# alevar/tiebrush

Measured on AMD Instinct MI355X. Metric: input alignment records/sec collapsed (tiebrush) + bases/sec covered (tiecov), higher is better.
Workload: dtype int64; 1 GPU; c3: 64 synthetic sorted BAMs x 5000000 100bp reads per GPU, --clip collapse + tiecov -c -j of the result; records_per_gpu=320000000, groups_out=25086541, parallelism=files-per-rank x1, ranks_seen=1, resident=SoA in HBM before the timed region, contexts=3

## Files before the change

### tiebrush_amd/csrc/collapse.hip

```cpp
#include <stdlib.h>

#include <chrono>

#include "cb_tiles.hpp"
#include "dev_common.hpp"
#include "rx_w64.hpp"
#include "scan_op.hpp"
#include "strategy.hpp"
#include "tbk_internal.h"
#include "wgroup.h"

namespace {

struct EffKey {
  uint32_t khi_h, khi_l;
  int32_t kend;
  uint32_t flag_cnt;
};
struct EffOp {
  __device__ __forceinline__ EffKey operator()(const EffKey& a, const EffKey& b) const {
    uint64_t ak = ((uint64_t)a.khi_h << 32) | a.khi_l, bk = ((uint64_t)b.khi_h << 32) | b.khi_l;
    bool take_b = (b.flag_cnt >> 31) || bk > ak || (bk == ak && b.kend > a.kend);
    EffKey r;
    r.khi_h = take_b ? b.khi_h : a.khi_h;
// ... 1915 lines not shown
      if (n_long && !literal) {
        hipStream_t keep = ctx->stream;
        if (aux) ctx->stream = aux;
        TBK_LAUNCH(ctx, "yd_wave", yd_wave_k, n_long, 64, 0, ids_long, n_wave, nchains, nit, chain_first, Y, YdWords{iv, io}, noff, ex_s, ex_e, J.g_yd,
                   yd_d, ids_over, n_over);
        ctx->stream = keep;
        if (aux) TBK_HIP(hipEventRecord(ctx->aux_done, aux));
      }
      if (n_lane && !literal)
        TBK_LAUNCH(ctx, "yd_lane", yd_lane_k<8>, cdiv(n_lane, 64), 64, 0, ids_lane, n_lane, nchains, nit, chain_first, Y, YdWords{iv, io}, ex_s, ex_e, J.g_yd,
                   yd_d, ids_over, n_over);
      if (n_long && aux) TBK_HIP(hipStreamWaitEvent(ctx->stream, ctx->aux_done, 0));
      TBK_LAUNCH(ctx, "yd_run_overflow", yd_run_k, cdiv(nchains, 64), 64, 0, ids_over, n_over, nchains, nit, chain_first, Y, YdWords{iv, io}, noff, ex_s, ex_e,
                 N, J.g_yd, yd_d);
    }
    if (by_list) {
      TBK_LAUNCH(ctx, "yd_gather", yd_lgather_k, ys_tiles, 512, 0, ng, ys_tiles, ys_table, ys_totals, yd_d, ys_item, J.gperm, J.G, J.cap, J.out_yd);
      TBK_HIP(hipStreamSynchronize(ctx->stream));
      if (ph)
        fprintf(stderr, "YD stage ms: counts %.1f | placement + numbering %.1f | buckets %.1f | list machines + gather %.1f (arena %.2f of %.2f GB, %zu overflow chunks)\n",
                std::chrono::duration<double, std::milli>(p1 - p0).count(), std::chrono::duration<double, std::milli>(p2 - p1).count(),
                std::chrono::duration<double, std::milli>(p3 - p2).count(), since(p3), ctx->ws_off / 1e9, ctx->ws_cap / 1e9, ctx->ws_overflow.size());
      return tbk_check_launch(ctx, "collapse_yd");
    }
  }
  TBK_LAUNCH(ctx, "col_write_yd", col_write_yd_k, cdiv(ng, B), B, 0, ng, J.gperm, J.G, J.g_yd, J.cap, J.out_yd);
  TBK_HIP(hipStreamSynchronize(ctx->stream));
  return tbk_check_launch(ctx, "collapse_yd");
}

int tbk_collapse_warm(tbk_ctx* ctx) {
  TBK_HIP(hipSetDevice(ctx->device));
  uint64_t* sc = ctx->d_scalars;
  TBK_HIP(hipMemsetAsync(sc, 0, 32 * sizeof(uint64_t), ctx->stream));
  TBK_HIP(hipStreamSynchronize(ctx->stream));
  uint32_t* z = (uint32_t*)sc;
  YdItems Y{};
  Y.pk = (uint4*)sc, Y.nex = z;
  const YdWords W{nullptr, z};
  const SegNodes N{z, z, (int32_t*)z};
  hipStream_t aux = tbk_aux_stream(ctx);
  if (aux) {
    hipStream_t keep = ctx->stream;
    ctx->stream = aux;
    TBK_LAUNCH(ctx, "yd_wave", yd_wave_k, 1, 64, 0, z, z, 0u, 0u, z, Y, W, z, z, z, (int32_t*)nullptr, z + 8, z + 16, z + 1);
    ctx->stream = keep;
    TBK_HIP(hipEventRecord(ctx->aux_done, aux));
    TBK_HIP(hipStreamWaitEvent(ctx->stream, ctx->aux_done, 0));
  } else {
    TBK_LAUNCH(ctx, "yd_wave", yd_wave_k, 1, 64, 0, z, z, 0u, 0u, z, Y, W, z, z, z, (int32_t*)nullptr, z + 8, z + 16, z + 1);
  }
  TBK_LAUNCH(ctx, "yd_lane", yd_lane_k<8>, 1, 64, 0, z, 0u, 0u, 0u, z, Y, W, z, z, (int32_t*)nullptr, z + 8, z + 16, z + 1);
  TBK_LAUNCH(ctx, "yd_run_overflow", yd_run_k, 1, 64, 0, z, z, 0u, 0u, z, Y, W, z, z, z, N, (int32_t*)nullptr, z + 8);
  TBK_HIP(hipStreamSynchronize(ctx->stream));
  return tbk_check_launch(ctx, "warmup");
}

int tbk_collapse_device(tbk_ctx* ctx, const tbk_collapse_opts* o, const tbk_soa_in* in, tbk_groups_out* out) {
  const uint32_t n = in->n_records;
  const uint32_t B = 256;
  out->n_groups = 0;
  out->n_passed = 0;
  ctx->route = tbk_collapse_route{};
  if (out->rec_group) TBK_HIP(hipMemsetAsync(out->rec_group, 0xFF, (size_t)n * 4, ctx->stream));
  if (n == 0) return 0;
  uint64_t* sc = ctx->d_scalars;
  ColIn I;
  I.n = n;
  I.k = in->n_files;
  {
    uint32_t* d_fo = ws_alloc<uint32_t>(ctx, in->n_files + 1);
    uint8_t* d_tb = ws_alloc<uint8_t>(ctx, in->n_files);
    if (!d_fo || !d_tb) return TBK_ENOMEM;
    const size_t fo_bytes = (size_t)(in->n_files + 1) * 4, tb_bytes = in->n_files;
    if (fo_bytes + tb_bytes <= 4096 * sizeof(uint64_t)) {
      char* stage = (char*)tbk_stage_acquire(ctx);
      memcpy(stage, in->file_off, fo_bytes);
      TBK_HIP(hipMemcpyAsync(d_fo, stage, fo_bytes, hipMemcpyHostToDevice, ctx->stream));
      if (in->tbmerged) {
        memcpy(stage + fo_bytes, in->tbmerged, tb_bytes);
        TBK_HIP(hipMemcpyAsync(d_tb, stage + fo_bytes, tb_bytes, hipMemcpyHostToDevice, ctx->stream));
      } else {
        TBK_HIP(hipMemsetAsync(d_tb, 0, tb_bytes, ctx->stream));
      }
      tbk_stage_release(ctx);
    } else {
      TBK_HIP(hipMemcpyAsync(d_fo, in->file_off, fo_bytes, hipMemcpyHostToDevice, ctx->stream));
      if (in->tbmerged) {
        TBK_HIP(hipMemcpyAsync(d_tb, in->tbmerged, tb_bytes, hipMemcpyHostToDevice, ctx->stream));
      } else {
        TBK_HIP(hipMemsetAsync(d_tb, 0, tb_bytes, ctx->stream));
      }
      TBK_HIP(hipStreamSynchronize(ctx->stream));
    }
    I.file_off = d_fo;
    I.tbm = d_tb;
  }
  I.tid = in->tid;
  I.pos = in->pos;
  I.flag = in->flag;
  I.mapq = in->mapq;
  I.strand = in->strand;
  I.nh = in->nh;
  I.cig_off = in->cig_off;
  I.cig = in->cig;
  I.yc_in = in->yc_in;
// ... 771 lines not shown
```

### tiebrush_amd/csrc/tbk_api.hip

```cpp
#include <sys/mman.h>

#include <algorithm>
#include <chrono>
#include <mutex>
#include <vector>
#include <new>

#include "tbk_internal.h"

namespace {
std::mutex g_reg_m;
struct RegEntry {
  void* p;
  int users;
};
std::vector<RegEntry> g_reg;
}

static void release_registered(tbk_ctx* ctx) {
  if (ctx->registered.empty()) return;
  (void)hipStreamSynchronize(ctx->stream);
  const auto r0 = std::chrono::steady_clock::now();
  struct RP {
    tbk_ctx* c;
// ... 401 lines not shown
}

static int yd_stage_on(tbk_ctx* run_on, void* job, size_t hint) {
  if (hipSetDevice(run_on->device) != hipSuccess) return TBK_EHIP;
  tbk_prof_begin_call(run_on);
  int rc = ws_begin_call(run_on, hint);
  if (rc == 0) rc = tbk_collapse_yd_run(run_on, job);
  tbk_prof_end_call(run_on);
  return rc;
}

static int finish_yd(tbk_ctx* ctx) {
  if (!ctx->yd_pending) return 0;
  ctx->yd_worker->wait();
  ctx->yd_pending = false;
  ctx->ws_base_off = 0;
  if (ctx->yd_ctx) {
    ctx->last_times = ctx->yd_ctx->last_times;
    if (ctx->yd_rc != 0) ctx->last_error = ctx->yd_ctx->last_error;
  }
  return ctx->yd_rc;
}

void tbk_debug_parse(const char* spec, TbkDebug* out) {
  *out = TbkDebug();
  if (!spec) return;
  std::string s(spec);
  size_t at = 0;
  while (at < s.size()) {
    size_t end = s.find(',', at);
    if (end == std::string::npos) end = s.size();
    const std::string kv = s.substr(at, end - at);
    at = end + 1;
    const size_t eq = kv.find('=');
    const std::string k = kv.substr(0, eq), v = eq == std::string::npos ? std::string("1") : kv.substr(eq + 1);
    const unsigned long long u = strtoull(v.c_str(), nullptr, 0);
    const bool on = v != "0";
    if (k == "path") out->path = v == "sort" ? 1 : (v == "window" ? 2 : 0);
    else if (k == "raw") out->raw = on ? 1 : 0;
    else if (k == "sort") out->sort = v == "radix" ? 1 : (v == "runs" ? 2 : 0);
    else if (k == "scan") out->scan = v == "lookback" ? 1 : (v == "3pass" ? 2 : 0);
    else if (k == "hash_mask") out->hash_mask = (uint32_t)u;
    else if (k == "qhash_mask") out->qhash_mask = u;
    else if (k == "yd_wave_min") out->yd_wave_min = (uint32_t)u;
    else if (k == "yd_bgrid") out->yd_bgrid = (uint32_t)u;
    else if (k == "yd_radix") out->yd_radix = on;
    else if (k == "yd_literal") out->yd_literal = on;
    else if (k == "yd_front") out->yd_front_split = v == "split";
    else if (k == "yd_own_arena") out->yd_own_arena = on;
    else if (k == "wg_stats") out->wg_stats = on;
    else if (k == "wg_og") out->wg_og = (uint32_t)u;
    else if (k == "wg_dense_verify") out->wg_dense_verify = on;
    else if (k == "wg_rank_merge") out->wg_rank_merge = on;
    else if (k == "cov_legacy") out->cov_legacy = on;
    else if (k == "cov_bundle_scan") out->cov_bundle_scan = on;
    else if (k == "cov_prep") out->cov_prep = on;
    else if (k == "cov_tile_cap") out->cov_tile_cap = u;
    else if (k == "junc_radix") out->junc_radix = on;
    else if (k == "no_junc_agg") out->no_junc_agg = on;
    else if (k == "jh_cap") out->jh_cap = (uint32_t)u;
    else if (k == "index_chain") out->index_chain = on;
    else if (k == "no_register") out->no_register = on;
    else if (k == "phases") out->phases = on;
    else if (k == "no_bounce") out->no_bounce = on;
    else if (k == "fmt_slice") out->fmt_slice = u;
  }
}

extern "C" {

int tbk_abi_version(void) { return TBK_ABI_VERSION; }

int tbk_set_debug(tbk_ctx* ctx, const char* spec) {
  if (!ctx) return TBK_EINVAL;
  tbk_debug_parse(spec, &ctx->dbg);
  if (ctx->yd_ctx) ctx->yd_ctx->dbg = ctx->dbg;
  if (ctx->side_ctx) ctx->side_ctx->dbg = ctx->dbg;
  return 0;
}

const char* tbk_strerror(int s) {
  switch (s) {
    case TBK_OK: return "ok";
    case TBK_EINVAL: return "invalid argument";
    case TBK_ENOMEM: return "out of memory";
    case TBK_EHIP: return "HIP runtime error";
    case TBK_E2BIG: return "output capacity too small";
    case TBK_EUNSUPPORTED: return "option or input outside the supported/pinned semantics";
    case TBK_EUNSORTED: return "input not coordinate-sorted";
    case TBK_EFATALOP: return "unknown opcode (tiecov accepts only M/I/D/N/S)";
    case TBK_ECOLLISION: return "key hash collision survived all reseeds";
    case TBK_ENODEVICE: return "no usable gfx950 device";
  }
  return "unknown status";
}

int tbk_create(int device_ordinal, tbk_ctx** out) {
  if (!out) return TBK_EINVAL;
  *out = nullptr;
  int ndev = 0;
  if (hipGetDeviceCount(&ndev) != hipSuccess || ndev <= 0 || device_ordinal < 0 || device_ordinal >= ndev) return TBK_ENODEVICE;
  tbk_ctx* ctx = new (std::nothrow) tbk_ctx();
  if (!ctx) return TBK_ENOMEM;
  ctx->device = device_ordinal;
  tbk_debug_parse(getenv("TBK_DEBUG"), &ctx->dbg);
  bool ok = hipSetDevice(device_ordinal) == hipSuccess;
// ... 476 lines not shown
```

### tiebrush_amd/csrc/tbk_internal.h

```cpp
#pragma once
#include <hip/hip_runtime.h>
#include <stdint.h>
#include <stdio.h>
#include <string.h>

#include <string>
#include <condition_variable>
#include <functional>
#include <mutex>
#include <thread>
#include <utility>
#include <vector>

#include "../../include/tbk.h"

enum : uint32_t {
  TBK_DERR_UNSORTED = 1u << 0,
  TBK_DERR_COLLISION = 1u << 1,
  TBK_DERR_FATALOP = 1u << 2,
  TBK_DERR_SPAN = 1u << 3,
  TBK_DERR_NCIGAR = 1u << 4,
  TBK_DERR_FRACTIONAL = 1u << 5,
  TBK_DERR_OVERFLOW = 1u << 6,
  TBK_DERR_INTERNAL = 1u << 7,
// ... 17 lines not shown
      std::lock_guard<std::mutex> lk(m);
      if (!started) {
        started = true;
        th = std::thread([this]() {
          std::unique_lock<std::mutex> lk2(m);
          for (;;) {
            cv.wait(lk2, [&] { return quit || (bool)job; });
            if (quit) return;
            std::function<void()> run = std::move(job);
            job = nullptr;
            lk2.unlock();
            run();
            lk2.lock();
            busy = false;
            cv.notify_all();
          }
        });
      }
      job = std::move(j);
      busy = true;
    }
    cv.notify_all();
  }
  void wait() {
    std::unique_lock<std::mutex> lk(m);
    cv.wait(lk, [&] { return !busy; });
  }
  ~TbkWorker() {
    {
      std::lock_guard<std::mutex> lk(m);
      quit = true;
    }
    cv.notify_all();
    if (th.joinable()) th.join();
  }
};

struct TbkDebug {
  int path = 0;
  int raw = -1;
  int sort = 0;
  int scan = 0;
  uint32_t hash_mask = 0xFFFFFFFFu;
  uint64_t qhash_mask = ~0ull;
  uint32_t yd_wave_min = 0;
  uint32_t yd_bgrid = 0;
  bool yd_radix = false;
  bool yd_literal = false;
  bool yd_front_split = false;
  bool yd_own_arena = false;
  uint32_t wg_og = 0;
  bool wg_stats = false;
  bool wg_dense_verify = false, wg_rank_merge = false;
  bool cov_legacy = false, cov_bundle_scan = false, cov_prep = false, junc_radix = false, no_junc_agg = false;
  uint64_t cov_tile_cap = 0;
  uint32_t jh_cap = 0;
  bool index_chain = false;
  bool no_register = false;
  bool no_bounce = false;
  bool phases = false;
  uint64_t fmt_slice = 0;
};
void tbk_debug_parse(const char* spec, TbkDebug* out);

struct tbk_ctx {
  int device = 0;
  TbkDebug dbg;
  hipStream_t own_stream = nullptr;
  hipStream_t stream = nullptr;
  hipStream_t aux = nullptr;
  hipEvent_t aux_done = nullptr;
  char* ws = nullptr;
  size_t ws_cap = 0, ws_off = 0;
  size_t ws_top = 0;
  bool ws_top_mode = false;
  bool ws_borrowed = false;
  std::vector<std::pair<char*, size_t>> ws_overflow;
  size_t ws_over_used = 0;
  uint32_t* d_err = nullptr;
  uint64_t* d_scalars = nullptr;
  uint64_t* h_scalars = nullptr;
  hipEvent_t stage_ev = nullptr;
  char* d_view = nullptr;
  size_t d_view_cap = 0;
  struct ViewPrep {
    bool valid = false;
    const void* cig = nullptr;
    uint32_t n = 0;
    int32_t *start = nullptr, *end = nullptr, *yi = nullptr;
    uint32_t *jcnt = nullptr, *ridx = nullptr;
    const void* agg = nullptr;
    uint32_t agg_tiles = 0;
    uint64_t n_bases = 0, sum_abs = 0, n_junc = 0;
    uint32_t err = 0;
  } view_prep;
  bool profiling = false;
  std::vector<KTime> ktimes;
  std::vector<hipEvent_t> ev_pool;
  size_t ev_used = 0;
  std::vector<tbk_kernel_time> last_times;
  std::string last_error;
  tbk_collapse_route route{};
  int num_cu = 256;
  void* yd_job = nullptr;
  tbk_ctx* yd_ctx = nullptr;
  TbkWorker* yd_worker = nullptr;
// ... 72 lines not shown
template <class T>
static inline T* ws_alloc(tbk_ctx* ctx, size_t n) {
  return (T*)tbk_ws_alloc_raw(ctx, n * sizeof(T));
}

hipEvent_t tbk_event(tbk_ctx* ctx);
static inline void tbk_prof_begin(tbk_ctx* ctx, const char* name) {
  if (!ctx->profiling) return;
  KTime k{name, tbk_event(ctx), tbk_event(ctx)};
  (void)hipEventRecord(k.a, ctx->stream);
  ctx->ktimes.push_back(k);
}
static inline void tbk_prof_end(tbk_ctx* ctx) {
  if (!ctx->profiling) return;
  (void)hipEventRecord(ctx->ktimes.back().b, ctx->stream);
}

#define TBK_LAUNCH(ctx, name, kern, grid, block, shmem, ...)                          \
  do {                                                                                \
    tbk_prof_begin(ctx, name);                                                        \
    hipLaunchKernelGGL(kern, dim3(grid), dim3(block), shmem, (ctx)->stream, __VA_ARGS__); \
    tbk_prof_end(ctx);                                                                \
  } while (0)

void tbk_prof_begin_call(tbk_ctx* ctx);
void tbk_prof_end_call(tbk_ctx* ctx);
int tbk_check_launch(tbk_ctx* ctx, const char* what);
extern "C" void tbk_bam_release(tbk_ctx* ctx);
void* tbk_stage_acquire(tbk_ctx* ctx);
void tbk_stage_release(tbk_ctx* ctx);
int tbk_sync_err(tbk_ctx* ctx, uint32_t* err_bits);
int tbk_derr_to_status(tbk_ctx* ctx, uint32_t bits);

static inline uint32_t cdiv(uint64_t a, uint64_t b) { return (uint32_t)((a + b - 1) / b); }

int tbk_exscan_u32(tbk_ctx* ctx, const uint32_t* in, uint32_t* out, uint32_t n, uint64_t* d_total);
int tbk_exscan_u32_u64(tbk_ctx* ctx, const uint32_t* in, uint64_t* out, uint32_t n, uint64_t* d_total);

struct SortBufs {
  uint64_t *hi, *lo;
  uint32_t* val;
  uint64_t *hi2, *lo2;
  uint32_t* val2;
};
int tbk_radix_sort128(tbk_ctx* ctx, SortBufs* b, uint32_t n, uint64_t only_hi = ~0ull, uint64_t only_lo = ~0ull,
                      bool masks_are_exact = false);
size_t tbk_radix_ws_bytes(uint32_t n);
int tbk_radix_sort_w64(tbk_ctx* ctx, uint64_t** w, uint64_t** w2, uint32_t n, uint64_t mask, bool mask_is_exact);
int tbk_sort_runs(tbk_ctx* ctx, SortBufs* b, uint32_t n_hi, const uint32_t* d_run_off, uint32_t nruns, uint32_t* err,
                  uint32_t* nbig_zeroed);

int tbk_collapse_device(tbk_ctx* ctx, const tbk_collapse_opts* o, const tbk_soa_in* in, tbk_groups_out* out);
int tbk_collapse_warm(tbk_ctx* ctx);
int tbk_collapse_yd_run(tbk_ctx* run_on, void* job);
int tbk_coverage_device(tbk_ctx* ctx, const tbk_cov_in* in, tbk_cov_out* out);
int tbk_cov_view_build(tbk_ctx* ctx, const int32_t* r_tid, const int32_t* r_pos, const uint8_t* r_strand, const uint32_t* r_cig_off,
                       const uint32_t* r_cig, const uint32_t* g_rep, const double* g_yc, const int64_t* g_yx, uint32_t ng, tbk_cov_in* view,
                       const uint64_t* g_key = nullptr);
int tbk_sample_device(tbk_ctx* ctx, const tbk_cov_in* in, int32_t num_samples, tbk_sample_out* out);
int tbk_format_device(tbk_ctx* ctx, const tbk_track_rows* rows, tbk_track_sink sink, void* user, uint64_t* out_bytes);
int tbk_names_upload(tbk_ctx* ctx, uint32_t n_names, const uint64_t* off, const char* bytes);
```

### tiebrush_amd/csrc/wgroup.hip

```cpp
#include <stdlib.h>

#include <algorithm>

#include "dev_common.hpp"
#include "strategy.hpp"
#include "tbk_internal.h"
#include "wgroup.h"

namespace {

constexpr int WG_NT = 512;
constexpr int WG_E = 8;
constexpr int WG_CAP = WG_NT * WG_E;
constexpr uint32_t WG_T = 1024;
constexpr uint32_t WG_KS = 2048;
constexpr int WG_NW = WG_NT / 64;
constexpr int WG_R = 4;
constexpr int WG_RS = 1;
constexpr int WG_RR = 1;

__global__ void wg_sample_k(const uint64_t* __restrict__ chi, uint32_t m, uint32_t s, uint32_t ns, uint64_t* __restrict__ shi) {
  uint32_t j = blockIdx.x * blockDim.x + threadIdx.x;
  if (j >= ns) return;
  uint64_t d = (uint64_t)j * s;
// ... 1542 lines not shown
    __syncthreads();
    for (uint32_t g = t; g < ng_w; g += WG_NT) {
      T.cnt[wbase + g] = gcnt[g];
      T.ns[wbase + g] = PART ? 0u : gns[g];
      T.rep[wbase + g] = grep[g];
      if constexpr (PART) {
        T.yx[wbase + g] = gns[g];
        T.yd[wbase + g] = gyd[g];
      }
    }
    if (t == 0) {
      T.wg_cnt[w] = ng_w;
      T.wp_cnt[w] = T.fmask ? 0u : np_w;
    }
    dbg_done(1, n_w);
    if (T.dbg && t == 0) {
      atomicAdd(&T.dbg[12], t_load - t_start);
      atomicAdd(&T.dbg[13], t_sort - t_load);
      atomicAdd(&T.dbg[14], t_heads - t_sort);
      atomicAdd(&T.dbg[15], __builtin_readcyclecounter() - t_heads);
    }
  }
}


__global__ __launch_bounds__(64) void wg_fmask_k(const uint32_t* __restrict__ ovf, uint32_t ovf_cap, WgTemp T) {
  const uint32_t cnt = ovf[0] < ovf_cap ? ovf[0] : ovf_cap;
  for (uint32_t wi = blockIdx.x; wi < cnt; wi += gridDim.x) {
    const uint32_t w = ovf[1 + wi];
    const uint32_t ng = T.wg_cnt[w], wb = T.wbase[w];
    for (uint32_t g = threadIdx.x; g < ng; g += 64) {
      const uint32_t p0 = T.poff[wb + g], n = T.ns[wb + g];
      uint64_t m = 0;
      for (uint32_t i = 0; i < n; ++i) m |= 1ull << (T.pinc[wb + p0 + i] & 0xFFFFu);
      T.fmask[wb + g] = m;
    }
  }
}
struct WgFinal {
  uint64_t* fmask;
  uint64_t *ghi, *glo;
  uint32_t *gmem, *gpoff, *pgrp, *first, *ns, *slot2sg;
  uint16_t* pfile;
  double* yc;
  long long *yxin, *ydin;
  unsigned long long* rep;
  uint8_t* tie;
  WgDirectOut D;
};
__global__ __launch_bounds__(256) void wg_compact_k(uint32_t nw, WgTemp T, const uint32_t* __restrict__ gbase, const uint32_t* __restrict__ pbase,
                                                   WgFinal F) {
  const uint32_t w = blockIdx.x * 4u + (threadIdx.x >> 6), lane = threadIdx.x & 63u;
  if (w >= nw) return;
  const uint32_t ng = T.wg_cnt[w], np = T.wp_cnt[w];
  if (!ng) return;
  const uint32_t wb = T.wbase[w], gb = gbase[w], pb = pbase[w];
  uint64_t c_hi = 0;
  uint32_t c_span = 0;
  for (uint32_t g = lane; g < ng; g += 64) {
    const uint32_t sg = gb + g;
    const uint64_t hi = T.hi[wb + g], lo = T.lo[wb + g];
    const uint32_t span = (uint32_t)(lo >> 32);
    uint64_t p_hi = __shfl_up((unsigned long long)hi, 1, 64);
    uint32_t p_span = __shfl_up(span, 1, 64);
    if (lane == 0) {
      p_hi = c_hi;
      p_span = c_span;
    }
    c_hi = __shfl((unsigned long long)hi, 63, 64);
    c_span = __shfl(span, 63, 64);
    const uint8_t tie = (g == 0 || hi != p_hi || span != p_span) ? 1 : 0;
    const unsigned long long r = T.rep[wb + g];
    const uint32_t cnt = T.cnt[wb + g], nsv = T.ns[wb + g];
    const uint64_t fm = F.fmask ? T.fmask[wb + g] : 0ull;
    const uint32_t po = F.fmask ? 0u : T.poff[wb + g];
    uint32_t yx = 0, yd = 0;
    if (F.yxin) {
      yx = T.yx[wb + g];
      yd = T.yd[wb + g];
    }
    F.ghi[sg] = hi;
    F.glo[sg] = lo;
    F.tie[sg] = tie;
    F.rep[sg] = r;
    F.gmem[sg] = (uint32_t)(r & 0xFFFFFFFFull);
    F.yc[sg] = (double)cnt;
    F.ns[sg] = nsv;
    if (F.yxin) {
      F.yxin[sg] = (long long)yx;
      F.ydin[sg] = (long long)yd;
    }
    F.first[sg] = sg;
    if (F.D.rep && sg < F.D.cap) {
      const int32_t st = (int32_t)(uint32_t)((hi >> 2) & 0x7FFFFFFFull);
      F.D.rep[sg] = (uint32_t)(r & 0xFFFFFFFFull);
      if (F.D.rep_effend) F.D.rep_effend[sg] = (int32_t)(uint32_t)(r >> 32);
      F.D.yc[sg] = (double)cnt;
      F.D.yx[sg] = (F.yxin ? (int64_t)yx : 0ll) + (int64_t)nsv;
      if (F.D.g_start) F.D.g_start[sg] = st;
      if (F.D.g_end) F.D.g_end[sg] = st + (int32_t)(uint32_t)(lo >> 32) - 1;
      if (F.D.g_key) {
        const uint32_t h32 = (uint32_t)lo;
        uint32_t shape = 0;
        if (F.D.strategy == TBK_STRAT_CIGAR || F.D.strategy == TBK_STRAT_CLIP) {
          if (h32 == (0x80000000u | C_M)) shape = 0x80000000u;
          if ((h32 >> 30) == 3u) shape = h32;
        }
        F.D.g_key[2 * (size_t)sg] = hi;
        F.D.g_key[2 * (size_t)sg + 1] = (lo & 0xFFFFFFFF00000000ull) | shape;
// ... 343 lines not shown
  ColIn I{};
  I.n = m;
  I.k = k;
  I.pos = r_pos;
  I.cig_off = cig_off;
  I.cig = cig;
  I.md_off = md_off;
  I.md = md;
  I.md_has = md_has;
  TBK_LAUNCH(ctx, "pr_merge", pr_merge_k, nw, PR_NT, 0, rows, off, k, nw, wbase, I, strategy, T, ctx->d_err);
  TBK_TRY(tbk_exscan_u32(ctx, T.wg_cnt, gbase, nw, sc + 1));
  uint32_t eb = 0;
  TBK_TRY(tbk_sync_err(ctx, &eb));
  if (eb & TBK_DERR_BIGBUCKET) {
    ctx->last_error = "more partials start on one base than a workgroup merges";
    return TBK_E2BIG;
  }
  if (eb) return tbk_derr_to_status(ctx, eb);
  const uint32_t ng = (uint32_t)ctx->h_scalars[1];
  out->n_groups = ng;
  if (ng > out->cap_groups) return TBK_E2BIG;
  if (ng == 0) return 0;
  uint64_t* okey = out->g_key;
  if (view && !okey) {
    okey = ws_alloc<uint64_t>(ctx, 2 * (size_t)ng);
    if (!okey) return TBK_ENOMEM;
  }
  TBK_LAUNCH(ctx, "pr_compact", pr_compact_k, cdiv(nw, 4u), 256, 0, nw, wbase, T, gbase, out->cap_groups, out->rep, out->yc, out->yx, out->yd,
             out->g_start, out->g_end, okey, strategy);
  if (view) return tbk_cov_view_build(ctx, r_tid, r_pos, r_strand, cig_off, cig, out->rep, out->yc, out->yx, ng, view, okey);
  TBK_HIP(hipStreamSynchronize(ctx->stream));
  return tbk_check_launch(ctx, "partial_reduce");
}


int tbk_window_groups(tbk_ctx* ctx, const tbkd::ColIn& I, int strategy, const uint64_t* chi, const uint64_t* clo, const uint32_t* cval,
                      const uint32_t* ceff, uint32_t m, const uint32_t* d_run_off, uint64_t* scratch_hi, uint64_t* scratch_lo,
                      bool want_rec_sg, uint64_t seed, WgOut* out, uint32_t* err_bits, const tbkd::ColOpt* raw_opt, bool part,
                      const WgDirectOut* direct) {
  const uint32_t k = I.k;
  const uint32_t B = 256;
  *err_bits = 0;
  const bool raw = raw_opt != nullptr;
  if (!tbk_window_supported(k) || m == 0) return TBK_EINVAL;
  if (part && (!raw || k > 64 || !I.prio_hi || !I.yc_in || !I.yx_in || !I.yd_in)) return TBK_EINVAL;
  struct TopMode {
    tbk_ctx* c;
    ~TopMode() {
      c->ws_top_mode = false;
      c->ws_top = 0;
    }
  } top_mode{ctx};
  ctx->ws_top_mode = true;
  WgRaw R{};
  unsigned long long* spread = nullptr;
  if (raw) {
    R.I = I;
    if (!R.I.cig) R.I.cig = R.I.cig_off;
    R.O = *raw_opt;
    R.O.seed = seed;
    spread = ws_alloc<unsigned long long>(ctx, 2 * (size_t)WG_NSPREAD * WG_SPREAD_STRIDE);
    if (!spread) return TBK_ENOMEM;
    TBK_HIP(hipMemsetAsync(spread, 0, 2 * (size_t)WG_NSPREAD * WG_SPREAD_STRIDE * sizeof(unsigned long long), ctx->stream));
    R.n_pass = spread;
    R.all_slots = want_rec_sg ? 1u : 0u;
    R.sparse = (!want_rec_sg && strategy != TBK_STRAT_FULL && !ctx->dbg.wg_dense_verify) ? 1u : 0u;
    R.n_slots = spread + (size_t)WG_NSPREAD * WG_SPREAD_STRIDE;
    scratch_hi = ws_alloc<uint64_t>(ctx, m);
    scratch_lo = ws_alloc<uint64_t>(ctx, m);
    if (!scratch_lo) return TBK_ENOMEM;
  }
  uint32_t s = 1;
  while (s * 2 * k <= WG_KS && s * 2 <= WG_T) s *= 2;
  const uint32_t g = WG_T / s;
  const uint32_t ns = cdiv(m, s);
  const uint32_t nsp = ns > 1 ? (ns - 1) / g : 0;
  const uint32_t nW = 2 * nsp;
  const uint32_t nw = nW + 1;
  const uint32_t nrows = nw + 1;
  uint64_t* W = ws_alloc<uint64_t>(ctx, nW + 1);
  uint32_t* off = ws_alloc<uint32_t>(ctx, (size_t)nrows * k);
  if (!W || !off) return TBK_ENOMEM;
  int32_t* ctid = nullptr;
  if (raw) {
    const uint32_t nchunks = cdiv(m, WG_TC);
    ctid = ws_alloc<int32_t>(ctx, nchunks);
    if (!ctid) return TBK_ENOMEM;
    TBK_LAUNCH(ctx, "wg_sample", wg_tidchunks_k, cdiv(nchunks, B), B, 0, I.tid, m, d_run_off, k, nchunks, ctid);
  }
  if (nsp) {
    uint64_t* Y = ws_alloc<uint64_t>(ctx, ns);
    uint64_t* Y2 = ws_alloc<uint64_t>(ctx, ns);
    if (!Y2) return TBK_ENOMEM;
    if (raw)
      TBK_LAUNCH(ctx, "wg_sample", wg_sample_raw_k, cdiv(ns, B), B, 0, I.tid, I.pos, ctid, m, s, ns, Y);
    else
      TBK_LAUNCH(ctx, "wg_sample", wg_sample_k, cdiv(ns, B), B, 0, chi, m, s, ns, Y);
    TBK_TRY(tbk_radix_sort_w64(ctx, &Y, &Y2, ns, ~0ull, false));
    TBK_LAUNCH(ctx, "wg_split", wg_split_k, cdiv(nsp, B), B, 0, Y, g, nsp, W);
  }
  WgTemp T;
  T.wbase = ws_alloc<uint32_t>(ctx, (size_t)nw + 1);
  if (!T.wbase) return TBK_ENOMEM;
  TBK_TRY(wg_offsets_build(ctx, raw, chi, I.tid, I.pos, ctid, d_run_off, k, m, W, nW, nrows, off, T.wbase));
  T.hi = scratch_hi;
  T.lo = scratch_lo;
  T.cnt = ws_alloc<uint32_t>(ctx, m);
  T.ns = ws_alloc<uint32_t>(ctx, m);
  T.poff = ws_alloc<uint32_t>(ctx, m);
  T.rep = ws_alloc<unsigned long long>(ctx, m);
  T.pinc = ws_alloc<uint32_t>(ctx, m);
  T.wg_cnt = ws_alloc<uint32_t>(ctx, nw);
  T.wp_cnt = ws_alloc<uint32_t>(ctx, nw);
  T.cslot = ws_alloc<uint32_t>(ctx, m);
  T.fmask = nullptr;
  if (raw && !part && k <= 64 && tbk_yd_by_list(ctx, k)) {
    T.fmask = ws_alloc<uint64_t>(ctx, m);
    if (!T.fmask) return TBK_ENOMEM;
  }
  T.vsrc = nullptr;
  T.vcnt = nullptr;
  if (raw && R.sparse) {
    T.vsrc = ws_alloc<uint32_t>(ctx, m);
    T.vcnt = ws_alloc<uint32_t>(ctx, nw);
    if (!T.vsrc || !T.vcnt) return TBK_ENOMEM;
    TBK_HIP(hipMemsetAsync(T.vcnt, 0, (size_t)nw * 4, ctx->stream));
  }
  T.c2r = ws_alloc<uint32_t>(ctx, m);
  uint32_t* gbase = ws_alloc<uint32_t>(ctx, nw);
  uint32_t* pbase = ws_alloc<uint32_t>(ctx, nw);
  T.dbg = nullptr;
  T.yx = T.yd = nullptr;
  if (part) {
    T.yx = ws_alloc<uint32_t>(ctx, m);
    T.yd = ws_alloc<uint32_t>(ctx, m);
    if (!T.yd) return TBK_ENOMEM;
  }
  if (!T.pinc || !pbase || !T.c2r) return TBK_ENOMEM;
  if (raw && !R.sparse) TBK_HIP(hipMemsetAsync(T.cslot, 0xFF, (size_t)m * 4, ctx->stream));
  WgIn In{chi, clo, cval, ceff, off, W, k, nw, ctx->dbg.wg_rank_merge ? 1u : 0u};
  const uint32_t nwords = cdiv(k, 32);
  const uint32_t gcap = (WG_LDS_HASH - (8u * k + 8u)) / (44u + 4u * nwords);
  const uint32_t lds_hash = gcap * (44u + 4u * nwords) + 8u * k + 8u;
  const uint32_t ovf_cap = nw;
  uint32_t* ovf = ws_alloc<uint32_t>(ctx, (size_t)ovf_cap + 1);
  uint32_t* ovf2 = ws_alloc<uint32_t>(ctx, (size_t)ovf_cap + 1);
  if (!ovf || !ovf2) return TBK_ENOMEM;
  TBK_HIP(hipMemsetAsync(ovf, 0, sizeof(uint32_t), ctx->stream));
  TBK_HIP(hipMemsetAsync(ovf2, 0, sizeof(uint32_t), ctx->stream));
  const uint32_t* ovf1_dbg = ovf;
  uint32_t* wlist = ws_alloc<uint32_t>(ctx, nw);
  if (!wlist) return TBK_ENOMEM;
  uint64_t* scw = ctx->d_scalars;
  TBK_HIP(hipMemsetAsync(scw + 3, 0, sizeof(uint64_t), ctx->stream));
  TBK_HIP(hipMemsetAsync(T.wg_cnt, 0, (size_t)nw * 4, ctx->stream));
  TBK_HIP(hipMemsetAsync(T.wp_cnt, 0, (size_t)nw * 4, ctx->stream));
  TBK_LAUNCH(ctx, "wg_list", wg_list_k, cdiv(nw, 1024u), 1024, 0, nw, T.wbase, wlist, (unsigned long long*)(scw + 3));
  {
    uint32_t eb0 = 0;
    TBK_TRY(tbk_sync_err(ctx, &eb0));
    if (eb0) {
      *err_bits = eb0;
      return 0;
    }
  }
  const uint32_t nw_live = (uint32_t)ctx->h_scalars[3];
  if (nw_live) {
#define WG_BY_STRATEGY(LAUNCH)          \
  switch (strategy) {                  \
    case TBK_STRAT_CIGAR:              \
      LAUNCH(TBK_STRAT_CIGAR);         \
      break;                           \
    case TBK_STRAT_FULL:               \
      LAUNCH(TBK_STRAT_FULL);          \
      break;                           \
    case TBK_STRAT_CLIP:               \
      LAUNCH(TBK_STRAT_CLIP);          \
      break;                           \
    default:                           \
      LAUNCH(TBK_STRAT_EXON);          \
      break;                           \
  }
#define WG_L_HASH(S) TBK_LAUNCH(ctx, "wg_hash", (wg_hash_k<true, S, 0>), nw_live, WG_NT, lds_hash, In, R, T, gcap, nwords, seed, wlist, ovf, ovf_cap, ctx->d_err)
#define WG_L_HASH64(S)                                                                                                                       \
  TBK_LAUNCH(ctx, "wg_hash", (wg_hash_k<true, S, WG_GC64>), nw_live, WG_NT, WG_GC64 * 52u + 8u * 64u + 8u, In, R, T, gcap, nwords, seed, wlist, ovf, \
             ovf_cap, ctx->d_err)
    if (part) {
      R.O.strategy = strategy;
      TBK_LAUNCH(ctx, "wg_hash", (wg_hash_k<true, -1, WG_GC64, true>), nw_live, WG_NT, WG_GC64 * 52u + 8u * 64u + 8u, In, R, T, gcap, nwords, seed, wlist,
                 ovf, ovf_cap, ctx->d_err);
    } else if (raw && k <= 64 && !T.dbg) {
      WG_BY_STRATEGY(WG_L_HASH64)
    } else if (raw) {
      WG_BY_STRATEGY(WG_L_HASH)
    } else {
      TBK_LAUNCH(ctx, "wg_hash", (wg_hash_k<false, -1, 0>), nw_live, WG_NT, lds_hash, In, R, T, gcap, nwords, seed, wlist, ovf, ovf_cap, ctx->d_err);
    }
    const uint32_t gcap2 = (WG_LDS_HASH2 - (8u * k + 8u)) / (44u + 4u * nwords);
    const uint32_t lds_hash2 = gcap2 * (44u + 4u * nwords) + 8u * k + 8u;
    if (gcap2 < 65536u) {
#define WG_L_HASH2(S)                                                                                                                      \
  TBK_LAUNCH(ctx, "wg_hash2", (wg_hash2_k<true, S, 0>), std::min<uint32_t>(nw_live, 512u), WG_NT, lds_hash2, In, R, T, gcap2, nwords, seed, ovf, ovf2, \
             ovf_cap, ctx->d_err)
#define WG_L_HASH2_64(S)                                                                                                                     \
  TBK_LAUNCH(ctx, "wg_hash2", (wg_hash2_k<true, S, WG_GC64_2>), std::min<uint32_t>(nw_live, 512u), WG_NT, WG_GC64_2 * 52u + 8u * 64u + 8u, In, R, \
             T, gcap2, nwords, seed, ovf, ovf2, ovf_cap, ctx->d_err)
      if (part) {
        TBK_LAUNCH(ctx, "wg_hash2", (wg_hash2_k<true, -1, WG_GC64_2, true>), std::min<uint32_t>(nw_live, 512u), WG_NT,
                   WG_GC64_2 * 52u + 8u * 64u + 8u, In, R, T, gcap2, nwords, seed, ovf, ovf2, ovf_cap, ctx->d_err);
      } else if (raw && k <= 64 && !T.dbg) {
        WG_BY_STRATEGY(WG_L_HASH2_64)
      } else if (raw) {
        WG_BY_STRATEGY(WG_L_HASH2)
      } else {
        TBK_LAUNCH(ctx, "wg_hash2", (wg_hash2_k<false, -1, 0>), std::min<uint32_t>(nw_live, 512u), WG_NT, lds_hash2, In, R, T, gcap2, nwords, seed, ovf,
                   ovf2, ovf_cap, ctx->d_err);
      }
      ovf = ovf2;
    }
  }
#define WG_L_SORT(S) TBK_LAUNCH(ctx, "wg_sort", (wg_sort_k<true, S>), std::min<uint32_t>(nw, 1024u), WG_NT, 0, In, R, T, I, strategy, ovf, ovf_cap, ctx->d_err)
  if (part) {
    TBK_LAUNCH(ctx, "wg_sort", (wg_sort_k<true, -1, true>), std::min<uint32_t>(nw, 1024u), WG_NT, 0, In, R, T, I, strategy, ovf, ovf_cap, ctx->d_err);
  } else if (raw) {
    WG_BY_STRATEGY(WG_L_SORT)
  } else {
    TBK_LAUNCH(ctx, "wg_sort", (wg_sort_k<false, -1>), std::min<uint32_t>(nw, 1024u), WG_NT, 0, In, R, T, I, strategy, ovf, ovf_cap, ctx->d_err);
  }
  if (T.fmask) TBK_LAUNCH(ctx, "wg_fmask", wg_fmask_k, std::min<uint32_t>(nw, 1024u), 64, 0, ovf, ovf_cap, T);
  uint64_t* sc = ctx->d_scalars;
  if (ctx->dbg.wg_stats) {
    TBK_HIP(hipMemcpyAsync(sc + 9, ovf1_dbg, sizeof(uint32_t), hipMemcpyDeviceToDevice, ctx->stream));
    TBK_HIP(hipMemcpyAsync(sc + 10, ovf2, sizeof(uint32_t), hipMemcpyDeviceToDevice, ctx->stream));
  }
  if (spread) TBK_LAUNCH(ctx, "wg_spread_sum", wg_spread_sum_k, 1, 64, 0, spread, (unsigned long long*)(sc + 0), (unsigned long long*)(sc + 6));
  TBK_TRY(tbk_exscan_u32(ctx, T.wg_cnt, gbase, nw, sc + 1));
  TBK_TRY(tbk_exscan_u32(ctx, T.wp_cnt, pbase, nw, sc + 2));
  uint32_t eb = 0;
  TBK_TRY(tbk_sync_err(ctx, &eb));
  *err_bits = eb;
  if (ctx->dbg.wg_stats) {
    ctx->route.wg_stats = 1;
    ctx->route.nw = nw;
    ctx->route.nw_live = nw_live;
    ctx->route.ovf1 = (uint32_t)ctx->h_scalars[9];
    ctx->route.ovf2 = (uint32_t)ctx->h_scalars[10];
  }
  if (T.dbg) {
    unsigned long long h[32];
    TBK_HIP(hipMemcpy(h, T.dbg, sizeof(h), hipMemcpyDeviceToHost));
    uint32_t o1 = 0, o2 = 0;
    TBK_HIP(hipMemcpy(&o1, ovf1_dbg, 4, hipMemcpyDeviceToHost));
    TBK_HIP(hipMemcpy(&o2, ovf, 4, hipMemcpyDeviceToHost));
    fprintf(stderr, "wg windows: %u with records, %u overflowed the first table (%u slots), %u the second\n", nw_live, o1, gcap, o2);
    static const char* ph[11] = {"prologue+init", "-", "key loads", "probe", "barrier 1", "atomics", "barrier 2", "-",
                                 "rank sort", "emit", "-"};
    unsigned long long tot = 0;
    for (int i = 0; i < 11; ++i) tot += h[16 + i];
    for (int i = 0; i < 11; ++i)
      fprintf(stderr, "wg_hash phase %-15s %8.1f Mcyc %5.1f %%\n", ph[i], h[16 + i] / 1e6, tot ? 100.0 * h[16 + i] / tot : 0.0);
    const char* nm[3] = {"empty", "sort", "hash"};
    fprintf(stderr, "wg_window lds phases (Mcyc): load %.1f  sort %.1f  heads+verify %.1f  reduce+write %.1f\n", h[12] / 1e6, h[13] / 1e6,
            h[14] / 1e6, h[15] / 1e6);
    for (int i = 0; i < 3; ++i)
      fprintf(stderr, "wg_window %-6s blocks %8llu records %10llu  cycles/block avg %9.0f max %9llu  (total %.1f Mcyc)\n", nm[i], h[i * 4 + 1],
              h[i * 4 + 2], h[i * 4 + 1] ? (double)h[i * 4] / (double)h[i * 4 + 1] : 0.0, h[i * 4 + 3], (double)h[i * 4] / 1e6);
  }
  if (eb) return 0;
  const uint32_t ng = (uint32_t)ctx->h_scalars[1], np = (uint32_t)ctx->h_scalars[2];
  out->ng = ng;
  out->np = np;
  ctx->ws_top_mode = false;
  out->ghi = ws_alloc<uint64_t>(ctx, ng);
  out->glo = ws_alloc<uint64_t>(ctx, ng);
  out->gmem = ws_alloc<uint32_t>(ctx, ng);
  out->gpoff = ws_alloc<uint32_t>(ctx, ng);
  out->gfmask = T.fmask ? ws_alloc<uint64_t>(ctx, ng) : nullptr;
  if (T.fmask && !out->gfmask) return TBK_ENOMEM;
  out->pfile = ws_alloc<uint16_t>(ctx, np);
  out->pgrp = tbk_yd_by_list(ctx, k) ? nullptr : ws_alloc<uint32_t>(ctx, np);
  out->yc = ws_alloc<double>(ctx, ng);
  out->ns = ws_alloc<uint32_t>(ctx, ng);
  out->yxin = part ? ws_alloc<long long>(ctx, ng) : nullptr;
  out->ydin = part ? ws_alloc<long long>(ctx, ng) : nullptr;
  if (part && !out->ydin) return TBK_ENOMEM;
  out->rep = ws_alloc<unsigned long long>(ctx, ng);
  out->first = ws_alloc<uint32_t>(ctx, ng);
  out->tie = ws_alloc<uint8_t>(ctx, ng);
  out->rec_sg = want_rec_sg ? ws_alloc<uint32_t>(ctx, I.n) : nullptr;
  ctx->ws_top_mode = true;
  uint32_t* slot2sg = want_rec_sg ? ws_alloc<uint32_t>(ctx, m) : nullptr;
  ctx->ws_top_mode = false;
  if (want_rec_sg && !slot2sg) return TBK_ENOMEM;
  if (!out->tie || (want_rec_sg && !out->rec_sg)) return TBK_ENOMEM;
  if (ng) {
    WgFinal F{out->gfmask, out->ghi, out->glo, out->gmem, out->gpoff, out->pgrp, out->first, out->ns, slot2sg, out->pfile, out->yc, out->yxin,
              out->ydin, out->rep, out->tie, (raw && direct) ? *direct : WgDirectOut{}};
    TBK_LAUNCH(ctx, "wg_compact", wg_compact_k, cdiv(nw, 4u), 256, 0, nw, T, gbase, pbase, F);
    if (want_rec_sg) TBK_HIP(hipMemsetAsync(out->rec_sg, 0xFF, (size_t)I.n * 4, ctx->stream));
    if (raw) {
      if (ctx->h_scalars[6] != 0 && R.sparse)
        TBK_LAUNCH(ctx, "wg_finish", wg_finish_sparse_k, cdiv(nw, 4u), 256, 0, nw, T.wbase, T.vcnt, T.vsrc, T.cslot, T.c2r, T.rep, I, strategy, ctx->d_err);
      else if (ctx->h_scalars[6] != 0)
        TBK_LAUNCH(ctx, "wg_finish", wg_finish_raw_k, cdiv(m, B), B, 0, m, T.cslot, T.c2r, T.rep, slot2sg, out->rec_sg, I, strategy, ctx->d_err);
    } else
      TBK_LAUNCH(ctx, "wg_finish", wg_finish_k, cdiv(m, B), B, 0, m, clo, cval, T.cslot, T.c2r, T.rep, slot2sg, out->rec_sg, I, strategy,
                 ctx->d_err);
  }
  return tbk_check_launch(ctx, "window_groups");
}
```

Before: 20.99 billion records/s.

## Overlap sparse verify finish on aux stream and skip unused pbase scan

The sparse wg_finish verify pass now runs on an auxiliary stream. It is forked after the first hash pass and works on a separate vcnt buffer, so it overlaps the second hash pass, the scans and compaction, and a second verify launch covers the overflow pass. When fmask is present, the per-window pbase/wp_cnt allocation, memset and exscan are skipped. A warmup launch of the verify kernel on the aux stream is also added. This removes serial tail work and one scan, at the cost of cross-stream ordering risk and a doubled vcnt buffer.

Result: slower. 20.67 billion records/s (-1.6%).

```diff
diff --git a/tiebrush_amd/csrc/collapse.hip b/tiebrush_amd/csrc/collapse.hip
--- a/tiebrush_amd/csrc/collapse.hip
+++ b/tiebrush_amd/csrc/collapse.hip
@@ -1991,6 +1991,7 @@
   }
   TBK_LAUNCH(ctx, "yd_lane", yd_lane_k<8>, 1, 64, 0, z, 0u, 0u, 0u, z, Y, W, z, z, (int32_t*)nullptr, z + 8, z + 16, z + 1);
   TBK_LAUNCH(ctx, "yd_run_overflow", yd_run_k, 1, 64, 0, z, z, 0u, 0u, z, Y, W, z, z, z, N, (int32_t*)nullptr, z + 8);
+  TBK_TRY(tbk_window_warm(ctx));
   TBK_HIP(hipStreamSynchronize(ctx->stream));
   return tbk_check_launch(ctx, "warmup");
 }
diff --git a/tiebrush_amd/csrc/tbk_api.hip b/tiebrush_amd/csrc/tbk_api.hip
--- a/tiebrush_amd/csrc/tbk_api.hip
+++ b/tiebrush_amd/csrc/tbk_api.hip
@@ -477,6 +477,7 @@
     else if (k == "wg_og") out->wg_og = (uint32_t)u;
     else if (k == "wg_dense_verify") out->wg_dense_verify = on;
     else if (k == "wg_rank_merge") out->wg_rank_merge = on;
+    else if (k == "wg_verify") out->wg_verify_serial = v == "serial";
     else if (k == "cov_legacy") out->cov_legacy = on;
     else if (k == "cov_bundle_scan") out->cov_bundle_scan = on;
     else if (k == "cov_prep") out->cov_prep = on;
diff --git a/tiebrush_amd/csrc/tbk_internal.h b/tiebrush_amd/csrc/tbk_internal.h
--- a/tiebrush_amd/csrc/tbk_internal.h
+++ b/tiebrush_amd/csrc/tbk_internal.h
@@ -93,6 +93,7 @@
   uint32_t wg_og = 0;
   bool wg_stats = false;
   bool wg_dense_verify = false, wg_rank_merge = false;
+  bool wg_verify_serial = false;
   bool cov_legacy = false, cov_bundle_scan = false, cov_prep = false, junc_radix = false, no_junc_agg = false;
   uint64_t cov_tile_cap = 0;
   uint32_t jh_cap = 0;
@@ -271,6 +272,7 @@
 
 int tbk_collapse_device(tbk_ctx* ctx, const tbk_collapse_opts* o, const tbk_soa_in* in, tbk_groups_out* out);
 int tbk_collapse_warm(tbk_ctx* ctx);
+int tbk_window_warm(tbk_ctx* ctx);
 int tbk_collapse_yd_run(tbk_ctx* run_on, void* job);
 int tbk_coverage_device(tbk_ctx* ctx, const tbk_cov_in* in, tbk_cov_out* out);
 int tbk_cov_view_build(tbk_ctx* ctx, const int32_t* r_tid, const int32_t* r_pos, const uint8_t* r_strand, const uint32_t* r_cig_off,
diff --git a/tiebrush_amd/csrc/wgroup.hip b/tiebrush_amd/csrc/wgroup.hip
--- a/tiebrush_amd/csrc/wgroup.hip
+++ b/tiebrush_amd/csrc/wgroup.hip
@@ -1618,9 +1618,9 @@
                                                    WgFinal F) {
   const uint32_t w = blockIdx.x * 4u + (threadIdx.x >> 6), lane = threadIdx.x & 63u;
   if (w >= nw) return;
-  const uint32_t ng = T.wg_cnt[w], np = T.wp_cnt[w];
+  const uint32_t ng = T.wg_cnt[w], np = pbase ? T.wp_cnt[w] : 0u;
   if (!ng) return;
-  const uint32_t wb = T.wbase[w], gb = gbase[w], pb = pbase[w];
+  const uint32_t wb = T.wbase[w], gb = gbase[w], pb = pbase ? pbase[w] : 0u;
   uint64_t c_hi = 0;
   uint32_t c_span = 0;
   for (uint32_t g = lane; g < ng; g += 64) {
@@ -2070,6 +2070,20 @@
     }
   } top_mode{ctx};
   ctx->ws_top_mode = true;
+  struct WgVerifyJoin {
+    tbk_ctx* c;
+    hipStream_t aux = nullptr;
+    hipError_t join() {
+      if (!aux) return hipSuccess;
+      hipError_t e = hipEventRecord(c->aux_done, aux);
+      if (e == hipSuccess) e = hipStreamWaitEvent(c->stream, c->aux_done, 0);
+      if (e == hipSuccess) aux = nullptr;
+      return e;
+    }
+    ~WgVerifyJoin() {
+      if (aux) (void)hipStreamSynchronize(aux);
+    }
+  } verify_join{ctx};
   WgRaw R{};
   unsigned long long* spread = nullptr;
   if (raw) {
@@ -2138,15 +2152,20 @@
   }
   T.vsrc = nullptr;
   T.vcnt = nullptr;
+  uint32_t *vcnt1 = nullptr, *vcnt2 = nullptr;
+  hipStream_t vaux = nullptr;
   if (raw && R.sparse) {
+    if (!ctx->dbg.wg_verify_serial) vaux = tbk_aux_stream(ctx);
     T.vsrc = ws_alloc<uint32_t>(ctx, m);
-    T.vcnt = ws_alloc<uint32_t>(ctx, nw);
-    if (!T.vsrc || !T.vcnt) return TBK_ENOMEM;
-    TBK_HIP(hipMemsetAsync(T.vcnt, 0, (size_t)nw * 4, ctx->stream));
+    vcnt1 = ws_alloc<uint32_t>(ctx, vaux ? 2 * (size_t)nw : (size_t)nw);
+    if (!T.vsrc || !vcnt1) return TBK_ENOMEM;
+    vcnt2 = vaux ? vcnt1 + nw : vcnt1;
+    TBK_HIP(hipMemsetAsync(vcnt1, 0, (vaux ? 2 * (size_t)nw : (size_t)nw) * 4, ctx->stream));
+    T.vcnt = vcnt1;
   }
   T.c2r = ws_alloc<uint32_t>(ctx, m);
   uint32_t* gbase = ws_alloc<uint32_t>(ctx, nw);
-  uint32_t* pbase = ws_alloc<uint32_t>(ctx, nw);
+  uint32_t* pbase = T.fmask ? nullptr : ws_alloc<uint32_t>(ctx, nw);
   T.dbg = nullptr;
   T.yx = T.yd = nullptr;
   if (part) {
@@ -2154,7 +2173,7 @@
     T.yd = ws_alloc<uint32_t>(ctx, m);
     if (!T.yd) return TBK_ENOMEM;
   }
-  if (!T.pinc || !pbase || !T.c2r) return TBK_ENOMEM;
+  if (!T.pinc || !gbase || (!T.fmask && !pbase) || !T.c2r) return TBK_ENOMEM;
   if (raw && !R.sparse) TBK_HIP(hipMemsetAsync(T.cslot, 0xFF, (size_t)m * 4, ctx->stream));
   WgIn In{chi, clo, cval, ceff, off, W, k, nw, ctx->dbg.wg_rank_merge ? 1u : 0u};
   const uint32_t nwords = cdiv(k, 32);
@@ -2172,7 +2191,7 @@
   uint64_t* scw = ctx->d_scalars;
   TBK_HIP(hipMemsetAsync(scw + 3, 0, sizeof(uint64_t), ctx->stream));
   TBK_HIP(hipMemsetAsync(T.wg_cnt, 0, (size_t)nw * 4, ctx->stream));
-  TBK_HIP(hipMemsetAsync(T.wp_cnt, 0, (size_t)nw * 4, ctx->stream));
+  if (pbase) TBK_HIP(hipMemsetAsync(T.wp_cnt, 0, (size_t)nw * 4, ctx->stream));
   TBK_LAUNCH(ctx, "wg_list", wg_list_k, cdiv(nw, 1024u), 1024, 0, nw, T.wbase, wlist, (unsigned long long*)(scw + 3));
   {
     uint32_t eb0 = 0;
@@ -2213,6 +2232,17 @@
       WG_BY_STRATEGY(WG_L_HASH)
     } else {
       TBK_LAUNCH(ctx, "wg_hash", (wg_hash_k<false, -1, 0>), nw_live, WG_NT, lds_hash, In, R, T, gcap, nwords, seed, wlist, ovf, ovf_cap, ctx->d_err);
+    }
+    if (vaux) {
+      hipEvent_t forked = tbk_event(ctx);
+      TBK_HIP(hipEventRecord(forked, ctx->stream));
+      TBK_HIP(hipStreamWaitEvent(vaux, forked, 0));
+      hipStream_t keep = ctx->stream;
+      ctx->stream = vaux;
+      verify_join.aux = vaux;
+      TBK_LAUNCH(ctx, "wg_finish", wg_finish_sparse_k, cdiv(nw, 4u), 256, 0, nw, T.wbase, vcnt1, T.vsrc, T.cslot, T.c2r, T.rep, I, strategy, ctx->d_err);
+      ctx->stream = keep;
+      T.vcnt = vcnt2;
     }
     const uint32_t gcap2 = (WG_LDS_HASH2 - (8u * k + 8u)) / (44u + 4u * nwords);
     const uint32_t lds_hash2 = gcap2 * (44u + 4u * nwords) + 8u * k + 8u;
@@ -2253,7 +2283,7 @@
   }
   if (spread) TBK_LAUNCH(ctx, "wg_spread_sum", wg_spread_sum_k, 1, 64, 0, spread, (unsigned long long*)(sc + 0), (unsigned long long*)(sc + 6));
   TBK_TRY(tbk_exscan_u32(ctx, T.wg_cnt, gbase, nw, sc + 1));
-  TBK_TRY(tbk_exscan_u32(ctx, T.wp_cnt, pbase, nw, sc + 2));
+  if (pbase) TBK_TRY(tbk_exscan_u32(ctx, T.wp_cnt, pbase, nw, sc + 2));
   uint32_t eb = 0;
   TBK_TRY(tbk_sync_err(ctx, &eb));
   *err_bits = eb;
@@ -2285,7 +2315,13 @@
               h[i * 4 + 2], h[i * 4 + 1] ? (double)h[i * 4] / (double)h[i * 4 + 1] : 0.0, h[i * 4 + 3], (double)h[i * 4] / 1e6);
   }
   if (eb) return 0;
-  const uint32_t ng = (uint32_t)ctx->h_scalars[1], np = (uint32_t)ctx->h_scalars[2];
+  if (verify_join.aux && ctx->h_scalars[6] != 0) {
+    hipStream_t keep = ctx->stream;
+    ctx->stream = verify_join.aux;
+    TBK_LAUNCH(ctx, "wg_finish", wg_finish_sparse_k, cdiv(nw, 4u), 256, 0, nw, T.wbase, vcnt2, T.vsrc, T.cslot, T.c2r, T.rep, I, strategy, ctx->d_err);
+    ctx->stream = keep;
+  }
+  const uint32_t ng = (uint32_t)ctx->h_scalars[1], np = pbase ? (uint32_t)ctx->h_scalars[2] : 0u;
   out->ng = ng;
   out->np = np;
   ctx->ws_top_mode = false;
@@ -2317,13 +2353,28 @@
     TBK_LAUNCH(ctx, "wg_compact", wg_compact_k, cdiv(nw, 4u), 256, 0, nw, T, gbase, pbase, F);
     if (want_rec_sg) TBK_HIP(hipMemsetAsync(out->rec_sg, 0xFF, (size_t)I.n * 4, ctx->stream));
     if (raw) {
-      if (ctx->h_scalars[6] != 0 && R.sparse)
-        TBK_LAUNCH(ctx, "wg_finish", wg_finish_sparse_k, cdiv(nw, 4u), 256, 0, nw, T.wbase, T.vcnt, T.vsrc, T.cslot, T.c2r, T.rep, I, strategy, ctx->d_err);
-      else if (ctx->h_scalars[6] != 0)
+      if (ctx->h_scalars[6] != 0 && R.sparse) {
+        if (!verify_join.aux)
+          TBK_LAUNCH(ctx, "wg_finish", wg_finish_sparse_k, cdiv(nw, 4u), 256, 0, nw, T.wbase, T.vcnt, T.vsrc, T.cslot, T.c2r, T.rep, I, strategy, ctx->d_err);
+      } else if (ctx->h_scalars[6] != 0)
         TBK_LAUNCH(ctx, "wg_finish", wg_finish_raw_k, cdiv(m, B), B, 0, m, T.cslot, T.c2r, T.rep, slot2sg, out->rec_sg, I, strategy, ctx->d_err);
     } else
       TBK_LAUNCH(ctx, "wg_finish", wg_finish_k, cdiv(m, B), B, 0, m, clo, cval, T.cslot, T.c2r, T.rep, slot2sg, out->rec_sg, I, strategy,
                  ctx->d_err);
   }
+  TBK_HIP(verify_join.join());
   return tbk_check_launch(ctx, "window_groups");
 }
+
+int tbk_window_warm(tbk_ctx* ctx) {
+  hipStream_t aux = tbk_aux_stream(ctx);
+  if (!aux) return 0;
+  hipStream_t keep = ctx->stream;
+  ctx->stream = aux;
+  TBK_LAUNCH(ctx, "wg_finish", wg_finish_sparse_k, 1, 256, 0, 0u, (const uint32_t*)nullptr, (const uint32_t*)nullptr, (const uint32_t*)nullptr,
+             (const uint32_t*)nullptr, (const uint32_t*)nullptr, (const unsigned long long*)nullptr, ColIn{}, (int)TBK_STRAT_CIGAR, ctx->d_err);
+  ctx->stream = keep;
+  TBK_HIP(hipEventRecord(ctx->aux_done, aux));
+  TBK_HIP(hipStreamWaitEvent(ctx->stream, ctx->aux_done, 0));
+  return tbk_check_launch(ctx, "window_warm");
+}
```
